# facebookresearch/fast3r

Hardware: AMD Instinct MI355X
Metric: views/sec (512^2, ViT-L) single forward pass at N=320 (higher is better)
Workload: dtype fp16

## Files before the change

### fast3r_amd/csrc/asm/attn_gen.py

```python
#!/usr/bin/env python3
import sys
import os

sys.path.insert(0, os.path.dirname(os.path.abspath(__file__)))
from isa import Program, Ins, Label, LabelRef, Lit, Neg, V, A, S, VCC, M0, EXEC, Reg

ARG_Q, ARG_O = 0, 8
ARG_LDQ = 16
ARG_NTILES = 32
ARG_QBS = 40
ARG_KVSHIFT = 56
ARG_STO = 64
ARG_KBS = 80
ARG_STLD = 96
ARG_TQ = 104
ARG_SEG = 112
SEG_BYTES = 24
ARG_DBG = ARG_SEG + 8 * SEG_BYTES
ARG_SCHED = ARG_DBG + 8
ARG_SIZE = ARG_SCHED + 32
FLAG_STATE_IN, FLAG_STATE_OUT = 1, 2

N_SLOTS = 4

s_q, s_k, s_vt, s_o = S(8, 2), S(10, 2), S(12, 2), S(14, 2)
s_ldq, s_ldk, s_ldvt, s_ldo = S(16), S(17), S(18), S(19)
s_nt, s_nseg = S(20), S(21)
s_wid, s_t, s_dma_u, s_seg_left = S(22), S(23), S(24), S(25)
s_kstep = S(26, 2)
s_m0base, s_seg, s_hopret, s_flags = S(28), S(29), S(30), S(31)
s_sto = S(32, 2)
s_lomask = S(34, 2)
s_ret, s_floor, s_ntm1 = S(36), S(37), S(38)
SEG0 = 52
s_stml = S(100, 2)


def seg_rec(i):
    return S(SEG0 + 6 * i, 2), S(SEG0 + 6 * i + 2, 2), S(SEG0 + 6 * i + 4)



s_delta = S(39)
s_shift = S(5)
s_tq = S(6)
s_rebase = S(7)
s_t0cyc, s_t0rt = S(SEG0 + 5), S(SEG0 + 11)

LANE = 0
s_mixrel = S(51)


class AttnGen:
    def __init__(self, dtype="f16", rowsum="pkadd", big_gap=None, k8_gap=2, name=None, ablate=(), cvt="rne", dma_aux="", dma_start=8, dma_step=None, pf=None, nslot=4,
                 fold="dot", head_dim=64, qk_planes=1, corr="f16", qk3_queues=True, k_hoist=True, qpw=None):
        assert dtype in ("f16", "bf16")
        assert head_dim in (64, 80, 128), "head widths with a generated kernel"
        assert qk_planes in (1, 2) and (qk_planes == 1 or (head_dim == 64 and dtype == "f16")) and corr in ("f16", "f8") and (corr == "f16" or qk_planes == 2)
        self.qk_planes, self.corr = qk_planes, corr
        self.qk3_queues = bool(qk3_queues)
        self.k_hoist = k_hoist
        self.dtype = dtype
        if rowsum == "pkadd" and dtype != "f16":
            rowsum = "add"
        self.rowsum = rowsum
        D = self.D = head_dim
        DK = self.DK = D * qk_planes
        assert qpw in (None, 2, 4) and (qpw is None or (head_dim == 64 and qk_planes == 1))
        self.QPW = QPW = qpw or (4 if (D == 64 and qk_planes == 1) else 2)
        self.WG_Q = 4 * QPW * 32
        self.NK = DK // 16
        self.QK_STEPS = ([(i, i) for i in range(self.NK)] if qk_planes == 1 else
                         [(i, i) for i in range(4)] + [(4 + i, i) for i in range(4)] + [(i, 4 + i) for i in range(4)])
        if corr == "f8":
            self.QK_STEPS = [(i, i) for i in range(4)] + [(6, 4, "f8", "unit", "lo"), (4, 6, "f8", "lo", "unit")]
        self.NQK = len(self.QK_STEPS)
        self.NDB = (D + 31) // 32
        self.DLAST = (D - 32 * (self.NDB - 1)) // 8
        self.KGROUPS = {64: [(0, 64)], 128: [(0, 64), (8192, 64)], 80: [(0, 64), (8192, 16)]}[DK]
        self.V_OFF = {64: 8192, 128: 16384, 80: 10240}[DK]
        self.SLOT = {64: 16384, 128: 32768, 80: 24576}[D] if qk_planes == 1 else 24576
        self.NP = 2 * (DK // 64) + (1 if D == 80 else 0) + 2 * (D // 64)
        if dma_step is None:
            dma_step = 6 if (D == 64 and qk_planes == 1 and self.QPW == 4) else 2
        self.dma_aux, self.dma_start, self.dma_step = dma_aux, dma_start, dma_step
        if pf is None:
            pf = 3 if corr == "f8" else 2
        assert nslot in (4, 8) and 2 <= pf <= nslot - 1
        assert D == 64 or nslot == 4
        self.pf, self.nslot = pf, nslot
        self.fold = fold
        self.LDS_X = nslot * self.SLOT
        self.lds_bytes = nslot * self.SLOT + 16
        v = 12
        self.S_BASE = v; v += 2 * QPW * 16
        self.P_BASE = v; v += QPW * 8
        self.NEGM = v; v += QPW * 16
        self.E_BASE = v; v += 4
        self.PSUM = v; v += QPW
        self.LRUN = v; v += QPW
        self.KCUR = v; v += 4
        self.VCUR = v; v += 4
        self.KREM = None
        if D == 80:
            self.KREM = v; v += 1
        self.SC_UNIT = self.SC_LO = None
        if corr == "f8":
            self.SC_UNIT = v; self.SC_LO = v + 1; v += 2
        a = 0
        self.O_BASE = a; a += QPW * self.NDB * 16
        self.Q_BASE = a; a += QPW * self.NK * 4
        self.KF_BASE = a; a += self.NK * 4
        self.VF_BASE = a; a += 2 * self.NDB * 4
        if a + self.NP <= 256:
            self.DOFF, self.doff_in_agpr = a, True
            a += self.NP
        else:
            self.DOFF, self.doff_in_agpr = v, False
            v += self.NP
        assert v <= 256 and a <= 256
        self.agpr_count = (a + 7) // 8 * 8
        pcs = []
        for goff, cols in self.KGROUPS:
            if cols == 64:
                pcs += [("A", "k", goff), ("A", "k", goff + 1024)]
        if D == 80:
            pcs.append(("A", "mix", None))
        for blk in range(D // 64):
            pcs += [("B", "vt", self.V_OFF + 8192 * blk), ("B", "vt", self.V_OFF + 8192 * blk + 1024)]
        assert len(pcs) == self.NP
        self.pieces = [(st, base, i, rel) for i, (st, base, rel) in enumerate(pcs)]
        if big_gap is None:
            big_gap = 4 if rowsum == "pkadd" else 5
        self.big_gap, self.k8_gap = (tuple(big_gap) if isinstance(big_gap, (tuple, list)) else (int(big_gap),)), k8_gap
        self.ablate = set(ablate)
        self.name = name or (f"f3r_attn_asm_q256_{dtype}" if (D == 64 and qk_planes == 1 and self.QPW == 2) else f"f3r_attn_asm_qk3f8_{dtype}" if corr == "f8" else f"f3r_attn_asm_qk3_{dtype}" if qk_planes == 2 else f"f3r_attn_asm_{dtype}" if D == 64 else f"f3r_attn_asm_d{D}_{dtype}")
        self.p = Program(self.name)
        if dtype == "f16":
            self.MFMA, self.MFMA8 = "v_mfma_f32_32x32x16_f16", "v_mfma_f32_32x32x8_f16"
            self.CVT, self.DOT, self.ONE2 = "v_cvt_pk_f16_f32", "v_dot2c_f32_f16", 0x3C003C00
            if cvt == "rtz":
                self.CVT = "v_cvt_pkrtz_f16_f32"
        else:
            self.MFMA, self.MFMA8 = "v_mfma_f32_32x32x16_bf16", "v_mfma_f32_32x32x8bf16_1k"
            self.CVT, self.DOT, self.ONE2 = "v_cvt_pk_bf16_f32", "v_dot2c_f32_bf16", 0x3F803F80

    def Sv(self, e, qb, r=None):
        base = self.S_BASE + e * self.QPW * 16 + qb * 16
        return V(base, 16) if r is None else V(base + r)

    def Pv(self, qb, ks, j=None):
        base = self.P_BASE + qb * 8 + ks * 4
        return V(base, 4) if j is None else V(base + j)

    def Nv(self, qb, r=None):
        base = self.NEGM + qb * 16
        return V(base, 16) if r is None else V(base + r)

    def Oa(self, qb, db, r=None):
        base = self.O_BASE + (qb * self.NDB + db) * 16
        return A(base, 16) if r is None else A(base + r)

    def Qa(self, qb, ds):
        return A(self.Q_BASE + (qb * self.NK + ds) * 4, 4)

    def KFa(self, ds):
        return A(self.KF_BASE + ds * 4, 4)

    def VFa(self, j):
# ... 244 lines not shown
            e("v_add_u32", V(6), S(40), V(6), comment="V^T row")
            e("v_lshrrev_b32", V(7), 1, V(6))
            e("v_and_b32", V(7), 7, V(7))
            e("v_xor_b32", V(7), V(7), V(10))
            e("v_lshlrev_b32", V(7), 4, V(7), comment="source chunk * 16")
            e("v_mul_lo_u32", V(6), V(6), s_ldvt)
            e("v_add_u32", V(6), V(6), V(7), comment="V^T rows 64..79: lane offset")
            e("s_cmp_lt_u32", s_wid, 2)
            e("s_cselect_b32", S(40), -1, 0)
            e("s_mov_b32", S(41), S(40))
            e("s_nop", 0)
            e("v_cndmask_b32", V(8), V(6), V(4), S(40, 2))
            park(mix, V(8))
            e("s_mov_b32", S(42), Lit(self.V_OFF + 8192 - 2048))
            e("s_cselect_b32", s_mixrel, Lit(self.KGROUPS[1][0]), S(42))
            e("s_lshl_b32", S(40), s_wid, 10)
            e("s_sub_u32", s_mixrel, s_mixrel, S(40), comment="destination of the mixed piece - s_m0base")
            for i in range(4):
                e("v_mov_b32", V(12 + i), 0)
            e("s_mul_i32", S(40), s_wid, Lit(self.SLOT))
            e("v_lshlrev_b32", V(8), 5, V(LANE))
            e("v_add_u32", V(8), S(40), V(8))
            e("ds_write_b128", V(8), V(12, 4), offset=self.V_OFF + 80 * 128)
            e("ds_write_b128", V(8), V(12, 4), offset=self.V_OFF + 80 * 128 + 16)
            e("s_waitcnt", "lgkmcnt(0)")
        e("s_lshl_b32", s_m0base, s_wid, 11, comment="slot 0 + wid * 2048")
        for i in range(self.pf):
            if i:
                e("s_add_u32", s_m0base, s_m0base, Lit(self.SLOT))
            self.emit_all(self.dma_pieces("A") + self.dma_pieces("B") + self.dma_advance())
            self.emit_all(self.seg_hop(i))
        e("s_add_u32", s_m0base, s_m0base, Lit(self.SLOT), comment="tile pf -> slot pf")
        self.emit_all(self.delta_for_tile())
        e("s_waitcnt", f"vmcnt({self.NP * (self.pf - 2)})", comment="tiles 0 and 1 have landed")
        e("s_barrier")
        for ds in range(NK):
            e_ = self.k_read(ds, 0)
            self.p.items.append(e_)
        e("s_waitcnt", "lgkmcnt(0)")
        self.emit_all(self.qk_mfmas(0))
        for ds in range(NK):
            self.p.items.append(self.k_read(ds, 1))

    def delta_for_tile(self):
        I = self.I
        msk = self.nslot - 1
        return [I("s_add_u32", S(40), s_t, 1), I("s_and_b32", S(40), S(40), msk), I("s_mov_b32", S(41), Lit((-msk * self.SLOT) & 0xFFFFFFFF)),
                I("s_cmp_eq_u32", S(40), 0), I("s_cselect_b32", s_delta, S(41), Lit(self.SLOT))]

    def own_rows_mask(self, qb):
        e = self.e
        e("s_sub_i32", S(46), s_shift, 32 * qb)
        e("v_cmp_le_i32", VCC, S(46), V(2))
        e("s_mov_b64", EXEC, VCC)

    def state_rows_offsets(self):
        e = self.e
        e("v_and_b32", V(2), 31, V(LANE), comment="lq")
        e("v_lshrrev_b32", V(3), 5, V(LANE), comment="g")
        e("s_load_dwordx2", S(44, 2), S(0, 2), Lit(ARG_STLD))
        e("s_waitcnt", "lgkmcnt(0)")
        e("v_mul_lo_u32", V(16), V(2), S(44))
        e("v_lshlrev_b32", V(1), 4, V(3))
        e("v_add_u32", V(16), V(16), V(1), comment="lq * st_o row stride + 16 g")
        e("v_mul_lo_u32", V(20), V(2), S(45))
        e("s_lshl_b32", S(46), S(44), 5)
        e("s_lshl_b32", S(47), S(45), 5)
# ... 34 lines not shown
            out += [I("s_nop", 0), I("global_load_lds_dwordx4", off, s_k if base == "k" else s_vt, **aux)]
        return out

    def dma_advance(self):
        I = self.I
        return [I("s_cmp_lt_u32", s_dma_u, s_ntm1),
                I("s_cselect_b32", S(40), s_kstep.sub(0), 0), I("s_cselect_b32", S(41), s_kstep.sub(1), 0),
                I("s_cselect_b32", S(42), 128, 0), I("s_cselect_b32", S(43), 1, 0),
                I("s_add_u32", s_k.sub(0), s_k.sub(0), S(40)), I("s_addc_u32", s_k.sub(1), s_k.sub(1), S(41)),
                I("s_add_u32", s_vt.sub(0), s_vt.sub(0), S(42)), I("s_addc_u32", s_vt.sub(1), s_vt.sub(1), 0),
                I("s_add_u32", s_dma_u, s_dma_u, S(43)),
                I("s_sub_u32", s_seg_left, s_seg_left, S(43))]

    def seg_hop(self, code):
        return [self.I("s_mov_b32", s_hopret, code), self.I("s_cmp_eq_u32", s_seg_left, 0), self.I("s_cbranch_scc1", self.L("NEXTSEG")),
                Label(f".L{self.name}_HOPRET_{code}")]

    def next_segment_block(self):
        e = self.e
        self.lab("NEXTSEG")
        e("s_add_u32", s_seg, s_seg, 1)
        for i in range(1, 8):
            e("s_cmp_eq_u32", s_seg, i)
            e("s_cbranch_scc1", self.L(f"SEG_{i}"))
        e("s_endpgm")
        for i in range(1, 8):
            k_i, vt_i, n_i = seg_rec(i)
            self.lab(f"SEG_{i}")
            e("s_mov_b64", s_k, k_i)
            e("s_mov_b64", s_vt, vt_i)
            e("s_mov_b32", s_seg_left, n_i)
            e("s_branch", self.L("SEG_DONE"))
        self.lab("SEG_DONE")
        for code in range(self.pf + 1):
            e("s_cmp_eq_u32", s_hopret, code)
            e("s_cbranch_scc1", self.L(f"HOPRET_{code}"))
        e("s_endpgm")

    def qk_mfmas(self, e_dst):
        out = []
        for step, st in enumerate(self.QK_STEPS):
            qf, kf = st[0], st[1]
            for qb in range(self.QPW):
                if len(st) == 2:
                    out.append(self.I(self.MFMA, self.Sv(e_dst, qb), self.KFa(kf), self.Qa(qb, qf), self.Nv(qb) if step == 0 else self.Sv(e_dst, qb)))
                else:
                    sc = {"unit": self.SC_UNIT, "lo": self.SC_LO}
                    out.append(self.I("v_mfma_scale_f32_32x32x64_f8f6f4", self.Sv(e_dst, qb), A(self.KF_BASE + kf * 4, 8), A(self.Q_BASE + (qb * self.NK + qf) * 4, 8),
                                      self.Sv(e_dst, qb), V(sc[st[3]]), V(sc[st[4]]), text="op_sel_hi:[0,0,0]"))
        return out

    def pv_mfmas(self, e_src=0):
        out = []
        for ks in range(2):
            for qb in range(self.QPW):
                for db in range(self.NDB):
                    out.append(self.I(self.MFMA, self.Oa(qb, db), self.VFa(ks * self.NDB + db), self.Pv(qb, ks), self.Oa(qb, db)))
        return out

    def softmax_flow(self, e):
        I = self.I
        QPW, NDB = self.QPW, self.NDB
        NPAIR = 8 * QPW
        flow = []
        first = 0 if QPW == 4 else 2
        E = lambda i, w: V(self.E_BASE + 2 * (i % 2) + w)

# ... 34 lines not shown
        if self.rowsum == "pkadd":
            red = ([I("v_pk_max_f16", V(1), V(PS), V(PS + 1)), I("v_pk_max_f16", V(2), V(PS + 2), V(PS + 3)), I("v_pk_max_f16", V(1), V(1), V(2))]
                   if self.QPW == 4 else [I("v_pk_max_f16", V(1), V(PS), V(PS + 1))])
            return [I("s_mov_b32", s_ret, ret_code)] + red + [
                    I("v_pk_max_f16", V(1), V(1), V(1), text="op_sel:[0,1] op_sel_hi:[1,0]"),
                    I("v_cmp_le_u32", VCC, Lit(0x50000000), V(1))] + ([] if "norare" in self.ablate else [
                    I("s_cbranch_vccnz", self.L(rare_label))])
        pad = [I("s_nop", 2)] if self.rowsum == "dot2c" else []
        red = ([I("v_max3_f32", V(1), V(PS), V(PS + 1), V(PS + 2)), I("v_max_f32", V(1), V(1), V(PS + 3))]
               if self.QPW == 4 else [I("v_max_f32", V(1), V(PS), V(PS + 1))])
        return [I("s_mov_b32", s_ret, ret_code)] + pad + red + [
                I("v_cmp_le_f32", VCC, 64.0, V(1))] + ([] if "norare" in self.ablate else [
                I("s_cbranch_vccnz", self.L(rare_label))])

    def l_adds(self):
        QPW, LRUN, PSUM = self.QPW, self.LRUN, self.PSUM
        if self.rowsum == "pkadd" and self.fold == "mix":
            out = []
            for half in (0, 1):
                for qb in range(QPW):
                    out.append(self.I("v_fma_mix_f32", V(LRUN + qb), V(PSUM + qb), 1.0, V(LRUN + qb),
                                      text=("op_sel:[1,0,0] " if half else "") + "op_sel_hi:[1,0,0]"))
            return out
        if self.rowsum == "pkadd":
            return [self.I(self.DOT, V(LRUN + qb), Lit(self.ONE2), V(PSUM + qb)) for qb in range(QPW)]
        return [self.I("v_add_f32", V(LRUN + qb), V(LRUN + qb), V(PSUM + qb)) for qb in range(QPW)]

    def addr_tail(self, is_a):
        I = self.I
        KCUR, VCUR = self.KCUR, self.VCUR
        regs = [KCUR + c for c in range(4)] + [VCUR, VCUR + 1] + ([self.KREM] if self.KREM is not None else []) if is_a else [VCUR + 2, VCUR + 3]
        return [I("v_add_u32", V(r), s_delta, V(r)) for r in regs]

    def stage(self, kind):
        I = self.I
        NK, NDB = self.NK, self.NDB
        is_a = kind.startswith("A")
        e_cur = 0 if is_a else 1
        e_nxt = 1 - e_cur
        has_qk = kind != "B_last"
        has_pv = kind != "A_first"
        do_sm = kind != "A_first"
        mf = (self.pv_mfmas() if has_pv else []) + (self.qk_mfmas(e_nxt) if has_qk else [])
        n_pv = 2 * self.QPW * NDB if has_pv else 0
        pinned = {i: [] for i in range(len(mf))}
        before = {i: [] for i in range(len(mf))}
        before[0].append(I("s_waitcnt", "lgkmcnt(0)"))
        hoist = self.corr == "f8" and self.qk3_queues and self.k_hoist
        if has_qk and has_pv:
            for ds in range(4 if hoist else 0, NK):
                pinned[ds - (4 if hoist else 0)].append(self.k_read(ds, 1 if is_a else 0))
            before[n_pv].append(I("s_waitcnt", "lgkmcnt(0)"))
        hoisted = [self.k_read(ds, 0 if is_a else 1) for ds in range(4)] if (hoist and has_qk) else []
        vbase = 0 if is_a else 2
        vreads = [I("ds_read_b128", self.VFa(ks * NDB + db), V(self.VCUR + vbase + ks), offset=db * 4096) for ks in range(2) for db in range(NDB)]
        tail = []
        if has_qk:
            for j, r in enumerate(vreads):
                pinned[n_pv + j].append(r)
        else:
            tail += vreads
        dma = (self.dma_pieces("A") if is_a else self.dma_pieces("B") + self.dma_advance()) if kind != "B_last" else []
        if "nodma" in self.ablate:
            dma = []
        tail += self.addr_tail(is_a)
        if kind == "B" and "nodma" not in self.ablate:
            tail += self.seg_hop(self.pf)
        flow = self.softmax_flow(e_cur) if do_sm else []
        if "nosoftmax" in self.ablate:
            flow = []
        two_queues = self.corr == "f8" and has_qk and has_pv and self.qk3_queues
        if not two_queues:
            flow = self.weave(flow, [(x, 0) for x in dma], start=self.dma_start, step=self.dma_step)
        if self.corr == "f8" and has_qk and has_pv and self.qk3_queues:
            n_last_read = n_pv + len(vreads)
            movable = [x for x in tail if getattr(x, "op", None) == "v_add_u32"]
            tail = [x for x in tail if getattr(x, "op", None) != "v_add_u32"]
            flow = flow + [(x, n_last_read) for x in movable]
            flow = flow + [(x, n_pv + 4 * self.QPW - 1) for x in hoisted]
            hoisted = []
        out = []
        fi = 0
        if two_queues:
            dq = list(dma)
            for i, m in enumerate(mf):
                out += before[i]
                out.append(m)
                took = len(pinned[i])
                out += pinned[i]
                cap = self.big_gap[i % len(self.big_gap)]
                if m.op.startswith("v_mfma_scale"):
                    cap = 2 * cap + 1
                gaps_left = len(mf) - i
                while took < cap:
                    flow_ok = fi < len(flow) and flow[fi][1] <= i
                    dma_due = dq and (not flow_ok or len(dq) > 3 * (gaps_left - 1))
                    if dma_due:
                        out.append(dq.pop(0))
                    elif flow_ok:
                        out.append(flow[fi][0])
# ... 225 lines not shown
        e("s_nop", 1)
        e("v_readfirstlane_b32", S(50), V(10))
        e("s_cmp_lt_u32", S(50), S(44))
        e("s_cbranch_scc0", self.L("F_EXIT"))
        e("s_mul_hi_u32", S(4), S(50), S(48))
        e("s_cmp_eq_u32", S(46), 1)
        e("s_cselect_b32", S(4), S(50), S(4), comment="z")
        e("s_mul_i32", S(51), S(4), S(46))
        e("s_sub_u32", S(51), S(50), S(51), comment="rem")
        e("s_mul_hi_u32", S(3), S(51), S(47))
        e("s_cmp_eq_u32", S(45), 1)
        e("s_cselect_b32", S(3), S(51), S(3), comment="y")
        e("s_mul_i32", S(2), S(3), S(45))
        e("s_sub_u32", S(2), S(51), S(2), comment="x")
        e("s_branch", self.L("WORK"))
        self.lab("F_EXIT")
        e("s_cmp_eq_u32", s_wid, 0)
        e("s_cbranch_scc0", self.L("F_END"))
        e("s_mov_b64", EXEC, 1)
        e("global_atomic_add", V(10), V(8), V(9), S(40, 2), offset=4, text="sc0")
        e("s_waitcnt", "vmcnt(0)")
        e("s_nop", 1)
        e("v_readfirstlane_b32", S(50), V(10))
        e("s_add_u32", S(50), S(50), 1)
        e("s_cmp_eq_u32", S(50), S(49))
        e("s_cbranch_scc0", self.L("F_END"))
        e("v_mov_b32", V(10), 0)
        e("v_mov_b32", V(11), 0)
        e("global_store_dwordx2", V(8), V(10, 2), S(40, 2), text="sc1")
        e("s_waitcnt", "vmcnt(0)")
        self.lab("F_END")
        e("s_endpgm")

    def build(self):
        p, e = self.p, self.e
        self.resume_labels = {0: [(0, "RESUME_A_FIRST"), (1, "RESUME_A")], 1: [(2, "RESUME_B"), (3, "RESUME_B_LAST")]}
        self.prologue()
        self.stage("A_first")
        e("s_mov_b32", s_ret, 0)
        e("s_branch", self.L("RARE_0"))
        self.lab("RESUME_A_FIRST")
        e("s_cmp_lt_u32", s_t, s_ntm1)
        e("s_cbranch_scc0", self.L("LAST_B"))
        p.items.append(Ins("s_nop", (0,), {}, "loop alignment"))
        self.lab("LOOP")
        self.stage("B")
        self.emit_all(self.check_block("RARE_1", 2))
        self.emit_all(self.l_adds())
        self.lab("RESUME_B")
        if "nobarrier" not in self.ablate:
            e("s_waitcnt", f"vmcnt({self.NP * (self.pf - 2)})")
            e("s_barrier")
        e("s_add_u32", s_t, s_t, 1)
        e("s_add_u32", S(40), s_t, self.pf)
        e("s_and_b32", S(40), S(40), self.nslot - 1)
        self.mul_const(S(40), S(40), self.SLOT)
        e("s_lshl_b32", S(41), s_wid, 11)
        e("s_add_u32", s_m0base, S(40), S(41), comment="LDS-DMA destination of tile t+pf")
        self.emit_all(self.delta_for_tile())
        self.stage("A")
        self.emit_all(self.check_block("RARE_0", 1))
        self.emit_all(self.l_adds())
        self.lab("RESUME_A")
        e("s_cmp_lt_u32", s_t, s_ntm1)
        e("s_cbranch_scc1", self.L("LOOP"))
        self.lab("LAST_B")
        self.stage("B_last")
        self.emit_all(self.check_block("RARE_1", 3))
        self.emit_all(self.l_adds())
        self.lab("RESUME_B_LAST")
        e("s_waitcnt", "lgkmcnt(0)")
        self.emit_all(self.pv_mfmas())
        self.epilogue()
        self.fetch_block()
        self.rare(0)
        self.rare(1)
        self.next_segment_block()
        return p

    def text(self):
        name = self.name
        body = self.p.body_text()
        return f"""
	.text
	.protected	{name}
	.globl	{name}
	.p2align	8
	.type	{name},@function
{name}:
{body}
.L{name}_end:
	.size	{name}, .L{name}_end-{name}
	.section	.rodata,"a",@progbits
	.p2align	6, 0x0
	.amdhsa_kernel {name}
		.amdhsa_group_segment_fixed_size {self.lds_bytes}
		.amdhsa_private_segment_fixed_size 0
		.amdhsa_kernarg_size {ARG_SIZE}
# ... 42 lines not shown
      - 2
      - 0
    .max_flat_workgroup_size: 256
    .name:           {self.name}
    .private_segment_fixed_size: 0
    .sgpr_count:     102
    .sgpr_spill_count: 0
    .symbol:         {self.name}.kd
    .uniform_work_group_size: 1
    .uses_dynamic_stack: false
    .vgpr_count:     {256 + self.agpr_count}
    .vgpr_spill_count: 0
    .wavefront_size: 64
"""


AttnGen2 = AttnGen


def module_text(gens):
    out = ['\t.amdgcn_target "amdgcn-amd-amdhsa--gfx950"\n\t.amdhsa_code_object_version 6\n']
    for g in gens:
        out.append(g.text())
    out.append("\t.amdgpu_metadata\n---\namdhsa.kernels:\n")
    for g in gens:
        out.append(g.metadata())
    out.append("amdhsa.target:   amdgcn-amd-amdhsa--gfx950\namdhsa.version:\n  - 1\n  - 2\n...\n\n\t.end_amdgpu_metadata\n")
    return "".join(out)


HEAD_DIMS = (64, 80, 128)


def product_generators(**kw):
    gens = []
    q3 = kw.pop("qk3_queues", True)
    kh = kw.pop("k_hoist", True)
    for hd in HEAD_DIMS:
        for dt in ("f16", "bf16"):
            g = AttnGen(dt, head_dim=hd, **kw)
            g.build()
            gens.append(g)
    kw3 = dict(kw)
    if kw3.get("dma_step") == 6:
        kw3["dma_step"] = None
    for dt in ("f16", "bf16"):
        g = AttnGen(dt, head_dim=64, qpw=2, **kw3)
        g.build()
        gens.append(g)
    for corr in ("f16", "f8"):
        g = AttnGen("f16", head_dim=64, qk_planes=2, corr=corr, qk3_queues=q3, k_hoist=kh, **kw3)
        g.build()
        gens.append(g)
    return gens


def main():
    import argparse
    ap = argparse.ArgumentParser()
    ap.add_argument("out")
    ap.add_argument("--rowsum", default="pkadd")
    ap.add_argument("--big-gap", default=None, help="fillers per MFMA gap: an int, or a comma list cycled over the gaps of a stage, e.g. 4,5")
    ap.add_argument("--k8-gap", type=int, default=2)
    ap.add_argument("--ablate", default="", help="comma list: nosoftmax,nodma,nobarrier,nolds,norare (timing only, wrong results)")
    ap.add_argument("--cvt", default="rne")
    ap.add_argument("--dma-aux", default="")
    ap.add_argument("--dma-start", type=int, default=8)
    ap.add_argument("--dma-step", type=int, default=6)
    ap.add_argument("--fold", default="dot")
    ap.add_argument("--layout", type=int, default=2, help="(accepted for old scripts; there is one layout)")
    ap.add_argument("--pf", type=int, default=None)
    ap.add_argument("--nslot", type=int, default=4)
    ap.add_argument("--qk3-queues", type=int, default=1, help="three-product kernels: 0 = in-order filler placement (measurement)")
    ap.add_argument("--k-hoist", type=int, default=1, help="fp8-correction kernel: 0 = K fragments requested in the stage that multiplies them (measurement)")
    a = ap.parse_args()
    bg = None if a.big_gap is None else (tuple(int(x) for x in a.big_gap.split(",")) if "," in a.big_gap else int(a.big_gap))
    gens = product_generators(rowsum=a.rowsum, big_gap=bg, k8_gap=a.k8_gap, ablate=[x for x in a.ablate.split(",") if x], cvt=a.cvt,
                              dma_aux=a.dma_aux, dma_start=a.dma_start, dma_step=a.dma_step, pf=a.pf, nslot=a.nslot, fold=a.fold, qk3_queues=bool(a.qk3_queues), k_hoist=bool(a.k_hoist))
    for g in gens:
        problems = g.p.check_hazards() if not a.ablate else []
        if problems:
            sys.stderr.write("\n".join(problems[:40]) + f"\n{len(problems)} hazard(s) in {g.name}\n")
            sys.exit(1)
    with open(a.out, "w") as f:
        f.write(module_text(gens))


if __name__ == "__main__":
    main()
```

### fast3r_amd/csrc/f3r_attn_asm.hip

```cpp
#include <cstddef>
#include <cstdlib>
#include <cstring>

#include "f3r_common.h"
#include "f3r_dispatch.h"

extern "C" const unsigned char f3r_attn_asm_hsaco[];
extern "C" const unsigned int f3r_attn_asm_hsaco_len;

namespace {

struct f3r_attn_asm_seg {
  const void* k;
  const void* vt;
  uint32_t tiles, pad;
};
struct f3r_attn_asm_args {
  const void* q;
  void* o;
  uint32_t ldq_b, ldk_b, ldvt_b, ldo_b;
  uint32_t n_tiles, n_seg;
  uint64_t q_bs, o_bs;
  uint32_t kv_shift, flags;
  float* st_o;
  float* st_ml;
  uint64_t k_bs, vt_bs;
  uint32_t st_o_ld_b, st_ml_ld_b;
  uint32_t tq, pad;
  f3r_attn_asm_seg seg[8];
  uint32_t* dbg;
  uint32_t* sched;
  uint32_t n_work, nx, nxy, nx_magic, nxy_magic, grid;
};
static_assert(sizeof(f3r_attn_asm_args) == 344 && offsetof(f3r_attn_asm_args, seg) == 112 && offsetof(f3r_attn_asm_args, dbg) == 304 &&
              offsetof(f3r_attn_asm_args, sched) == 312 && offsetof(f3r_attn_asm_args, n_work) == 320,
              "must match ARG_SIZE / ARG_SEG / ARG_DBG / ARG_SCHED of attn_gen.py");

constexpr int kNumHd = 3, kHd[kNumHd] = {64, 80, 128};
int hd_index(int hd) {
  for (int i = 0; i < kNumHd; ++i)
    if (kHd[i] == hd) return i;
  return -1;
}
AttnItem native_item(int hd, int planes) { return (hd == 64 && planes < 2) ? ATTN_ITEM_512 : ATTN_ITEM_256; }

F3rCodeObject<10> g_kernels = {f3r_attn_asm_hsaco,
                               {"f3r_attn_asm_f16", "f3r_attn_asm_bf16", "f3r_attn_asm_d80_f16", "f3r_attn_asm_d80_bf16", "f3r_attn_asm_d128_f16", "f3r_attn_asm_d128_bf16",
                                "f3r_attn_asm_qk3_f16", "f3r_attn_asm_qk3f8_f16", "f3r_attn_asm_q256_f16", "f3r_attn_asm_q256_bf16"}};

hipFunction_t get_fn(int dtype, int hi, int planes, AttnItem item) {
  if (dtype < 0 || dtype > 1 || hi < 0) return nullptr;
  const bool hd64 = kHd[hi] == 64;
  if (planes >= 2) return (hd64 && dtype == F3R_F16) ? g_kernels.get(4 + planes) : nullptr;
  if (item != native_item(kHd[hi], planes)) return hd64 ? g_kernels.get(8 + dtype) : nullptr;
  return g_kernels.get(2 * hi + dtype);
}

bool pow2(int x) { return x > 0 && (x & (x - 1)) == 0; }

bool q256_wins(int64_t tq, int64_t hb, int64_t cus) {
  const int64_t n512 = (tq + 511) / 512 * hb, n256 = (tq + 255) / 256 * hb;
  const double t512 = (double)((n512 + cus - 1) / cus), t256 = 0.64 * (double)((n256 + cus - 1) / cus);
  return t256 < 0.97 * t512;
}

int64_t tail_split_rows(int64_t tq, int64_t hb, int64_t cus) {
  const int64_t nqb = (tq + 511) / 512;
  if (nqb * hb <= cus) return 0;
  int64_t x = cus, y = hb;
  while (y) { const int64_t t = x % y; x = y; y = t; }
  const int64_t g = cus / x;
  const int64_t nqb_main = nqb / g * g;
  if (nqb_main == 0 || nqb_main == nqb) return 0;
  if (nqb_main * hb / cus > 8) return 0;
  const int64_t r = (nqb - nqb_main) * hb;
  if (2 * r > cus) return 0;
  return nqb_main * 512;
}

void plan_launches(const f3r_attn_args& a, AttnPlan& p) {
  const int hd = kHd[p.hd_index];
  p.main.rows = a.tq;
  p.main.item = native_item(hd, p.planes);
  if (p.main.item != ATTN_ITEM_512 || get_fn(a.dtype, p.hd_index, p.planes, ATTN_ITEM_256) == nullptr) return;
  static const char* force = getenv("F3R_ATTN_Q256");
  static const char* split = getenv("F3R_ATTN_TAIL_SPLIT");
  if (force && (force[0] == '0' || force[0] == '1')) {
    if (force[0] == '1') p.main.item = ATTN_ITEM_256;
    return;
  }
  const int64_t cus = f3r_device_cus(), hb = (int64_t)a.n_heads * a.batch;
  const bool may_split = !(split && split[0] == '0') && !a.state_in && !a.state_out && a.reserve_cus <= 0;
  const int64_t rows = may_split ? tail_split_rows(a.tq, hb, cus) : 0;
  if (rows > 0) {
    const AttnItem item = q256_wins(a.tq - rows, hb, cus) ? ATTN_ITEM_256 : ATTN_ITEM_512;
    if (a.tq - rows >= attn_item_wave_rows(item)) {
      p.main.rows = rows;
      p.tail.rows = a.tq - rows;
      p.tail.item = item;
      return;
    }
  }
  if (q256_wins(a.tq, hb, cus)) p.main.item = ATTN_ITEM_256;
}

}

bool f3r_attn_asm_plan(const f3r_attn_args& a, int64_t min_keys, AttnPlan* plan, const char** why) {
  *why = "";
  const int hd = a.head_dim == 0 ? 64 : a.head_dim;
  const int hi = hd_index(hd);
  if (hi < 0) { *why = "no generated kernel for this head_dim (64, 80, 128)"; return false; }
  const int qkp = a.qk_planes >= 2 ? a.qk_planes : 1;
  if (qkp >= 2 && (hd != 64 || a.dtype != F3R_F16)) { *why = "qk_planes 2 / 3 need head_dim 64 and fp16"; return false; }
  const int64_t wrows = attn_item_wave_rows(native_item(hd, qkp));
  if (a.causal) { *why = "causal mask"; return false; }
  if (!a.q_prescaled) { *why = "q not pre-scaled"; return false; }
  if (a.tq < wrows) { *why = "fewer query rows than one wave takes (128 at head_dim 64, 64 otherwise)"; return false; }
  if (a.kv_group > 1 && !pow2(a.kv_group)) { *why = "kv_group not a power of two"; return false; }
  if ((a.state_in || a.state_out) && a.batch != 1 && qkp < 2) { *why = "carried softmax state with batch > 1"; return false; }
  int first = -1;
  int64_t keys = 0;
  for (int s = 0; s < a.n_seg; ++s) {
    if (a.seg_len[s] == 0) continue;
    if (a.seg_len[s] % 64 != 0) { *why = "a K/V segment is not a multiple of 64 keys"; return false; }
    if (first < 0) first = s;
    if (a.ldvt[s] != a.ldvt[first] || a.k_batch_stride[s] != a.k_batch_stride[first] || a.vt_batch_stride[s] != a.vt_batch_stride[first]) {
      *why = "K/V segments with different ldvt / batch strides";
      return false;
    }
    keys += a.seg_len[s];
  }
  if (first < 0) { *why = "no keys"; return false; }
  if (keys < min_keys) { *why = "fewer keys than F3R_ATTN_ASM_MIN_KEYS"; return false; }
  if (keys / 64 >= (1ll << 31)) { *why = "too many keys"; return false; }
  if (wrows * a.ldq * 2 >= (1ll << 32) || wrows * a.ldo * 2 >= (1ll << 32) || 64 * a.ldk * 2 >= (1ll << 32) || (int64_t)hd * a.ldvt[first] * 2 >= (1ll << 32) ||
      wrows * a.n_heads * hd * 4 >= (1ll << 32)) {
    *why = "row strides too large for 32-bit lane offsets";
    return false;
  }
  if (a.tq >= (1ll << 31) || a.n_heads >= 65536 || a.batch >= 65536) { *why = "grid too large"; return false; }
  if (get_fn(a.dtype, hi, qkp, native_item(hd, qkp)) == nullptr) { *why = "the embedded code object could not be loaded on this device"; return false; }
  plan->family = ATTN_ASM;
  plan->hd_index = hi;
  plan->planes = qkp;
  plan_launches(a, *plan);
  return true;
}

const char* f3r_attn_asm_name(const f3r_attn_args& a, const AttnPlan& p) {
  const bool h = a.dtype == F3R_F16;
  if (p.planes == 2) return "f3r_attn_asm_qk3_f16 (hand-scheduled, three products per score block, csrc/asm/attn_gen.py)";
  if (p.planes == 3) return "f3r_attn_asm_qk3f8_f16 (hand-scheduled, three products per score block, the corrections on the fp8 MFMA, csrc/asm/attn_gen.py)";
  if (kHd[p.hd_index] == 80) return h ? "f3r_attn_asm_d80_f16 (hand-scheduled, csrc/asm/attn_gen.py)" : "f3r_attn_asm_d80_bf16 (hand-scheduled, csrc/asm/attn_gen.py)";
  if (kHd[p.hd_index] == 128) return h ? "f3r_attn_asm_d128_f16 (hand-scheduled, csrc/asm/attn_gen.py)" : "f3r_attn_asm_d128_bf16 (hand-scheduled, csrc/asm/attn_gen.py)";
  if (p.tail.rows > 0)
    return h ? "f3r_attn_asm_f16 + f3r_attn_asm_q256_f16 for the last round (hand-scheduled, csrc/asm/attn_gen.py)"
             : "f3r_attn_asm_bf16 + f3r_attn_asm_q256_bf16 for the last round (hand-scheduled, csrc/asm/attn_gen.py)";
  if (p.main.item == ATTN_ITEM_256)
    return h ? "f3r_attn_asm_q256_f16 (hand-scheduled, 256-query work items, csrc/asm/attn_gen.py)" : "f3r_attn_asm_q256_bf16 (hand-scheduled, 256-query work items, csrc/asm/attn_gen.py)";
  return h ? "f3r_attn_asm_f16 (hand-scheduled, csrc/asm/attn_gen.py)" : "f3r_attn_asm_bf16 (hand-scheduled, csrc/asm/attn_gen.py)";
}

static int launch_one(const f3r_attn_args& a, const AttnPlan& p, int64_t row0, const AttnAsmLaunch& l, hipStream_t stream) {
  const int hd = kHd[p.hd_index];
  const int wave_rows = attn_item_wave_rows(l.item);
  F3R_REQUIRE(l.rows >= wave_rows, "f3r_attn_fwd: a hand-scheduled launch of %lld query rows, fewer than the %d of one wave", (long long)l.rows, wave_rows);
  hipFunction_t fn = get_fn(a.dtype, p.hd_index, p.planes, l.item);
  if (!fn) {
    f3r_set_error("f3r_attn_fwd: the embedded hand-scheduled kernel could not be loaded on this device");
    return F3R_ERR_LAUNCH;
  }
  f3r_attn_asm_args k;
  memset(&k, 0, sizeof(k));
  k.q = (const char*)a.q + row0 * a.ldq * 2;
  k.o = (char*)a.o + row0 * a.ldo * 2;
  k.ldq_b = (uint32_t)(a.ldq * 2);
  k.ldk_b = (uint32_t)(a.ldk * 2);
  k.ldo_b = (uint32_t)(a.ldo * 2);
  k.q_bs = (uint64_t)a.q_batch_stride * 2;
  k.o_bs = (uint64_t)a.o_batch_stride * 2;
  int sh = 0;
  for (int gsz = a.kv_group > 1 ? a.kv_group : 1; gsz > 1; gsz >>= 1) ++sh;
  k.kv_shift = (uint32_t)sh;
  k.flags = (a.state_in ? 1u : 0u) | (a.state_out ? 2u : 0u);
  k.st_o = a.st_o;
  k.st_ml = a.st_ml;
  k.st_o_ld_b = (uint32_t)a.n_heads * (uint32_t)hd * 4u;
  k.st_ml_ld_b = (uint32_t)a.n_heads * 16u;
  k.tq = (uint32_t)l.rows;
  k.dbg = a.dbg_counters;
  for (int s = 0; s < a.n_seg; ++s) {
    if (a.seg_len[s] == 0) continue;
    f3r_attn_asm_seg& g = k.seg[k.n_seg++];
    g.k = a.k_seg[s];
    g.vt = a.vt_seg[s];
    g.tiles = (uint32_t)(a.seg_len[s] / 64);
    k.n_tiles += g.tiles;
    k.ldvt_b = (uint32_t)(a.ldvt[s] * 2);
    k.k_bs = (uint64_t)a.k_batch_stride[s] * 2;
    k.vt_bs = (uint64_t)a.vt_batch_stride[s] * 2;
// ... 40 lines not shown
```

### fast3r_amd/csrc/f3r_dispatch.h

```cpp
#pragma once
#include <atomic>
#include <map>
#include <mutex>

#include "f3r_common.h"

inline bool al16(const void* p) { return (((uintptr_t)p) & 15) == 0; }
inline bool al8(const void* p) { return (((uintptr_t)p) & 7) == 0; }

inline int f3r_device_cus() {
  static std::atomic<int> cache[64];
  int dev = 0, cu = 0;
  if (hipGetDevice(&dev) != hipSuccess) dev = 0;
  std::atomic<int>* slot = (dev >= 0 && dev < 64) ? &cache[dev] : nullptr;
  if (slot && (cu = slot->load(std::memory_order_relaxed)) != 0) return cu;
  if (hipDeviceGetAttribute(&cu, hipDeviceAttributeMultiprocessorCount, dev) != hipSuccess || cu < 8) cu = 256;
  if (slot) slot->store(cu, std::memory_order_relaxed);
  return cu;
}
inline int f3r_num_cus() { return f3r_device_cus() / 8 * 8; }

template <int N>
struct F3rCodeObject {
  const unsigned char* image;
// ... 64 lines not shown
  const int64_t rounds = (tiles + slots - 1) / slots;
  return eff * (float)tiles / (float)(rounds * slots);
}
inline float score_256(const f3r_gemm_args& a, int nh) {
  return tile_score(((a.M + 255) / 256) * ((a.N + 128 * nh - 1) / (128 * nh)), 256, nh == 2 ? 1.0f : 0.82f);
}
inline float score_128(const f3r_gemm_args& a) { return tile_score(((a.M + 127) / 128) * ((a.N + 127) / 128), 512, 0.72f); }

inline int f3r_gemm256_halves(const f3r_gemm_args& a, int forced) {
  if (a.epi == F3R_EPI_QKV) return 2;
  if (a.N % 256 != 0 || forced == 1) return 1;
  if (forced == 2) return 2;
  return score_256(a, 1) > score_256(a, 2) ? 1 : 2;
}
inline bool f3r_gemm256_preferred(const f3r_gemm_args& a) { return score_256(a, f3r_gemm256_halves(a, 0)) >= score_128(a); }

enum {
  ATTN_SEL_AUTO = 0,
  ATTN_SEL_HIP = 1,
  ATTN_SEL_ASM = 2,
};
enum AttnFamily {
  ATTN_HIP_CAUSAL,
  ATTN_HIP_BATCHED,
  ATTN_HIP,
  ATTN_GENERIC,
  ATTN_ASM,
};
enum AttnItem {
  ATTN_ITEM_512,
  ATTN_ITEM_256,
};
inline int attn_item_wave_rows(AttnItem item) { return item == ATTN_ITEM_512 ? 128 : 64; }
struct AttnAsmLaunch { int64_t rows = 0; AttnItem item = ATTN_ITEM_512; };
struct AttnPlan {
  AttnFamily family = ATTN_HIP;
  int hd_index = 0;
  int planes = 1;
  AttnAsmLaunch main, tail;
};
int f3r_attn_plan(const f3r_attn_args& a, AttnPlan* plan);
bool f3r_attn_asm_plan(const f3r_attn_args& a, int64_t min_keys, AttnPlan* plan, const char** why);
int f3r_attn_asm_launch(const f3r_attn_args& a, const AttnPlan& plan, hipStream_t stream);
const char* f3r_attn_asm_name(const f3r_attn_args& a, const AttnPlan& plan);
int f3r_attn_generic_launch(const f3r_attn_args& a, hipStream_t stream);
```

### include/f3r.h

```cpp
#ifndef F3R_H_
#define F3R_H_

#include <stddef.h>
#include <stdint.h>

#ifdef __cplusplus
extern "C" {
#endif

typedef void* f3r_stream_t;

typedef enum {
  F3R_OK = 0,
  F3R_ERR_ARG = -1,
  F3R_ERR_UNSUPPORTED = -2,
  F3R_ERR_LAUNCH = -3
} f3r_status;

typedef enum { F3R_F16 = 0, F3R_BF16 = 1 } f3r_dtype;
typedef enum { F3R_REAL_F32 = 0, F3R_REAL_F64 = 1 } f3r_real;
typedef enum { F3R_LOSS_DIS = 0, F3R_LOSS_LOG1P = 1 } f3r_loss_dis_mode;

#define F3R_MAX_SEG 8

// ... 86 lines not shown
  void* o;
  int64_t ldq, ldo;
  int64_t q_batch_stride, o_batch_stride;
  int64_t tq;
  int32_t batch;
  int32_t n_heads;
  int32_t n_seg;
  int32_t dtype;
  const void* k_seg[F3R_MAX_SEG];
  const void* vt_seg[F3R_MAX_SEG];
  int64_t seg_len[F3R_MAX_SEG];
  int64_t ldvt[F3R_MAX_SEG];
  int64_t ldk;
  int64_t k_batch_stride[F3R_MAX_SEG];
  int64_t vt_batch_stride[F3R_MAX_SEG];
  float scale;
  int32_t q_prescaled;
  float* st_o;
  float* st_ml;
  int32_t state_in;
  int32_t state_out;
  int32_t kv_group;
  int32_t causal;
  int64_t q_pos0;
  int64_t seg_pos0[F3R_MAX_SEG];
  int32_t kernel_sel;
  int32_t head_dim;
  uint32_t* dbg_counters;
  uint32_t* sched_counter;
  int32_t qk_planes;
  int32_t reserve_cus;
} f3r_attn_args;
#define F3R_ATTN_ASM_MIN_KEYS 2048

int f3r_attn_fwd(const f3r_attn_args* args, f3r_stream_t stream);
const char* f3r_attn_kernel_name(const f3r_attn_args* args);

int f3r_upsample2x(const void* in, const void* in_lo, void* out, void* out_lo, int batch, int h, int w, int C, int out_h, int out_w,
                   int dtype, f3r_stream_t stream);
int f3r_interp_bilinear(const void* in, const void* in_lo, void* out, void* out_lo, int batch, int h, int w, int C, int full_h, int full_w,
                        int out_h, int out_w, int dtype, f3r_stream_t stream);
int f3r_interp_bilinear_f8(const void* in, const void* in_lo, void* out, void* out_lo, void* out_f8, int batch, int h, int w, int C, int full_h,
                           int full_w, int out_h, int out_w, int dtype, f3r_stream_t stream);

typedef enum { F3R_DEPTH_EXP = 0, F3R_DEPTH_LINEAR = 1, F3R_DEPTH_SQUARE = 2 } f3r_depth_mode;
typedef enum { F3R_CONF_EXP = 0, F3R_CONF_SIGMOID = 1 } f3r_conf_mode;
int f3r_dpt_final(const void* x, const void* x_lo, const float* w, const float* b, int n_out, float* pts3d, float* conf, int64_t npix,
                  int Cin, int depth_mode, int conf_mode, float conf_vmin, float conf_vmax, int dtype, f3r_stream_t stream);

int f3r_cast_f32_to_lp(const float* in, void* out, void* out_lo, int64_t n, int dtype, f3r_stream_t stream);

size_t f3r_align_workspace_bytes(int n_prob);
int f3r_align_local_to_global(const float* conf, const float* pts_local, const float* pts_global, const uint8_t* valid_mask,
                              float* out, float* rts, float* thr_out, void* workspace, size_t ws_bytes, int n_prob,
                              int64_t npix, float quantile, f3r_stream_t stream);

size_t f3r_focal_workspace_bytes(int n_views, int H, int W);
int f3r_estimate_focal(const float* pts3d, const float* conf, float* focal, float* thr_out, void* workspace, size_t ws_bytes,
                       int n_views, int H, int W, float quantile, float ppx, float ppy, int n_iter, float min_focal, float max_focal,
                       f3r_stream_t stream);

size_t f3r_nn_index_bytes(int64_t m);
size_t f3r_nn_workspace_bytes(int64_t n);
int f3r_nn_build(const float* pts, int64_t m, void* index, size_t index_bytes, void* workspace, size_t ws_bytes, f3r_stream_t stream);
int f3r_nn_query(const void* index, const float* query, int64_t n, double* dist, int32_t* idx, void* workspace, size_t ws_bytes,
                 f3r_stream_t stream);
// ... 142 lines not shown
```

Before: 35.82.

## Add grouped attention kernel with one barrier per group of key tiles

```diff
diff --git a/fast3r_amd/csrc/asm/attn_gen.py b/fast3r_amd/csrc/asm/attn_gen.py
--- a/fast3r_amd/csrc/asm/attn_gen.py
+++ b/fast3r_amd/csrc/asm/attn_gen.py
@@ -53,7 +53,7 @@
 
 class AttnGen:
     def __init__(self, dtype="f16", rowsum="pkadd", big_gap=None, k8_gap=2, name=None, ablate=(), cvt="rne", dma_aux="", dma_start=8, dma_step=None, pf=None, nslot=4,
-                 fold="dot", head_dim=64, qk_planes=1, corr="f16", qk3_queues=True, k_hoist=True, qpw=None):
+                 fold="dot", head_dim=64, qk_planes=1, corr="f16", qk3_queues=True, k_hoist=True, qpw=None, tiles_per_barrier=1):
         assert dtype in ("f16", "bf16")
         assert head_dim in (64, 80, 128), "head widths with a generated kernel"
         assert qk_planes in (1, 2) and (qk_planes == 1 or (head_dim == 64 and dtype == "f16")) and corr in ("f16", "f8") and (corr == "f16" or qk_planes == 2)
@@ -86,8 +86,12 @@
         self.dma_aux, self.dma_start, self.dma_step = dma_aux, dma_start, dma_step
         if pf is None:
             pf = 3 if corr == "f8" else 2
-        assert nslot in (4, 8) and 2 <= pf <= nslot - 1
+            if tiles_per_barrier > 1:
+                pf = tiles_per_barrier + 1
+        G = self.G = int(tiles_per_barrier)
+        assert nslot in (4, 8) and G >= 1 and G + 1 <= pf and pf + G <= nslot, "LDS ring: G + 1 <= pf (read after write) and pf + G <= nslot (write after read)"
         assert D == 64 or nslot == 4
+        assert G == 1 or (D == 64 and qk_planes == 1 and self.QPW == 4)
         self.pf, self.nslot = pf, nslot
         self.fold = fold
         self.LDS_X = nslot * self.SLOT
@@ -135,6 +139,8 @@
         self.big_gap, self.k8_gap = (tuple(big_gap) if isinstance(big_gap, (tuple, list)) else (int(big_gap),)), k8_gap
         self.ablate = set(ablate)
         self.name = name or (f"f3r_attn_asm_q256_{dtype}" if (D == 64 and qk_planes == 1 and self.QPW == 2) else f"f3r_attn_asm_qk3f8_{dtype}" if corr == "f8" else f"f3r_attn_asm_qk3_{dtype}" if qk_planes == 2 else f"f3r_attn_asm_{dtype}" if D == 64 else f"f3r_attn_asm_d{D}_{dtype}")
+        if name is None and G > 1:
+            self.name += "_grp"
         self.p = Program(self.name)
         if dtype == "f16":
             self.MFMA, self.MFMA8 = "v_mfma_f32_32x32x16_f16", "v_mfma_f32_32x32x8_f16"
@@ -445,7 +451,10 @@
             self.emit_all(self.seg_hop(i))
         e("s_add_u32", s_m0base, s_m0base, Lit(self.SLOT), comment="tile pf -> slot pf")
         self.emit_all(self.delta_for_tile())
-        e("s_waitcnt", f"vmcnt({self.NP * (self.pf - 2)})", comment="tiles 0 and 1 have landed")
+        if self.G == 1:
+            e("s_waitcnt", f"vmcnt({self.NP * (self.pf - 2)})", comment="tiles 0 and 1 have landed")
+        else:
+            e("s_waitcnt", f"vmcnt({self.NP * (self.pf - 1 - self.G)})", comment=f"tiles 0 .. {self.G} have landed")
         e("s_barrier")
         for ds in range(NK):
             e_ = self.k_read(ds, 0)
@@ -546,7 +555,7 @@
             e("s_mov_b32", s_seg_left, n_i)
             e("s_branch", self.L("SEG_DONE"))
         self.lab("SEG_DONE")
-        for code in range(self.pf + 1):
+        for code in range(self.pf + self.G):
             e("s_cmp_eq_u32", s_hopret, code)
             e("s_cbranch_scc1", self.L(f"HOPRET_{code}"))
         e("s_endpgm")
@@ -647,7 +656,7 @@
         regs = [KCUR + c for c in range(4)] + [VCUR, VCUR + 1] + ([self.KREM] if self.KREM is not None else []) if is_a else [VCUR + 2, VCUR + 3]
         return [I("v_add_u32", V(r), s_delta, V(r)) for r in regs]
 
-    def stage(self, kind):
+    def stage(self, kind, hop_code=None):
         I = self.I
         NK, NDB = self.NK, self.NDB
         is_a = kind.startswith("A")
@@ -680,7 +689,7 @@
             dma = []
         tail += self.addr_tail(is_a)
         if kind == "B" and "nodma" not in self.ablate:
-            tail += self.seg_hop(self.pf)
+            tail += self.seg_hop(self.pf if hop_code is None else hop_code)
         flow = self.softmax_flow(e_cur) if do_sm else []
         if "nosoftmax" in self.ablate:
             flow = []
@@ -972,17 +981,8 @@
         self.lab("F_END")
         e("s_endpgm")
 
-    def build(self):
-        p, e = self.p, self.e
-        self.resume_labels = {0: [(0, "RESUME_A_FIRST"), (1, "RESUME_A")], 1: [(2, "RESUME_B"), (3, "RESUME_B_LAST")]}
-        self.prologue()
-        self.stage("A_first")
-        e("s_mov_b32", s_ret, 0)
-        e("s_branch", self.L("RARE_0"))
-        self.lab("RESUME_A_FIRST")
-        e("s_cmp_lt_u32", s_t, s_ntm1)
-        e("s_cbranch_scc0", self.L("LAST_B"))
-        p.items.append(Ins("s_nop", (0,), {}, "loop alignment"))
+    def plain_loop(self):
+        e = self.e
         self.lab("LOOP")
         self.stage("B")
         self.emit_all(self.check_block("RARE_1", 2))
@@ -1004,6 +1004,55 @@
         self.lab("RESUME_A")
         e("s_cmp_lt_u32", s_t, s_ntm1)
         e("s_cbranch_scc1", self.L("LOOP"))
+
+    def grouped_loop(self):
+        e = self.e
+        G = self.G
+        self.lab("LOOP")
+        for k in range(G):
+            code_a, code_b = (1, 2) if k == 0 else (2 + 2 * k, 3 + 2 * k)
+            self.stage("B", hop_code=self.pf + k)
+            self.emit_all(self.check_block("RARE_1", code_b))
+            self.emit_all(self.l_adds())
+            self.lab("RESUME_B" if k == 0 else f"RESUME_B_{k}")
+            if k == G - 1 and "nobarrier" not in self.ablate:
+                e("s_waitcnt", f"vmcnt({self.NP * (self.pf - 1 - G)})", comment=f"this wave's pieces of tiles .. t+1+{G} have landed")
+                e("s_barrier")
+            e("s_add_u32", s_t, s_t, 1)
+            e("s_add_u32", S(40), s_t, self.pf)
+            e("s_and_b32", S(40), S(40), self.nslot - 1)
+            self.mul_const(S(40), S(40), self.SLOT)
+            e("s_lshl_b32", S(41), s_wid, 11)
+            e("s_add_u32", s_m0base, S(40), S(41), comment="LDS-DMA destination of tile t+pf")
+            self.emit_all(self.delta_for_tile())
+            self.stage("A")
+            self.emit_all(self.check_block("RARE_0", code_a))
+            self.emit_all(self.l_adds())
+            self.lab("RESUME_A" if k == 0 else f"RESUME_A_{k}")
+            e("s_cmp_lt_u32", s_t, s_ntm1)
+            if k < G - 1:
+                e("s_cbranch_scc0", self.L("LAST_B"))
+            else:
+                e("s_cbranch_scc1", self.L("LOOP"))
+
+    def build(self):
+        p, e = self.p, self.e
+        self.resume_labels = {0: [(0, "RESUME_A_FIRST"), (1, "RESUME_A")], 1: [(2, "RESUME_B"), (3, "RESUME_B_LAST")]}
+        for k in range(1, self.G):
+            self.resume_labels[0].append((2 + 2 * k, f"RESUME_A_{k}"))
+            self.resume_labels[1].append((3 + 2 * k, f"RESUME_B_{k}"))
+        self.prologue()
+        self.stage("A_first")
+        e("s_mov_b32", s_ret, 0)
+        e("s_branch", self.L("RARE_0"))
+        self.lab("RESUME_A_FIRST")
+        e("s_cmp_lt_u32", s_t, s_ntm1)
+        e("s_cbranch_scc0", self.L("LAST_B"))
+        p.items.append(Ins("s_nop", (0,), {}, "loop alignment"))
+        if self.G > 1:
+            self.grouped_loop()
+        else:
+            self.plain_loop()
         self.lab("LAST_B")
         self.stage("B_last")
         self.emit_all(self.check_block("RARE_1", 3))
@@ -1112,13 +1161,16 @@
 HEAD_DIMS = (64, 80, 128)
 
 
-def product_generators(**kw):
+GROUPED_RING = dict(tiles_per_barrier=2, pf=4, nslot=8)
+
+
+def product_generators(ring=None, **kw):
     gens = []
     q3 = kw.pop("qk3_queues", True)
     kh = kw.pop("k_hoist", True)
     for hd in HEAD_DIMS:
         for dt in ("f16", "bf16"):
-            g = AttnGen(dt, head_dim=hd, **kw)
+            g = AttnGen(dt, head_dim=hd, **(dict(kw, name=f"f3r_attn_asm_{dt}", **ring) if (ring and hd == 64) else kw))
             g.build()
             gens.append(g)
     kw3 = dict(kw)
@@ -1130,6 +1182,10 @@
         gens.append(g)
     for corr in ("f16", "f8"):
         g = AttnGen("f16", head_dim=64, qk_planes=2, corr=corr, qk3_queues=q3, k_hoist=kh, **kw3)
+        g.build()
+        gens.append(g)
+    for dt in ("f16", "bf16"):
+        g = AttnGen(dt, head_dim=64, **dict(kw, name=f"f3r_attn_asm_{dt}_grp", **(ring or GROUPED_RING)))
         g.build()
         gens.append(g)
     return gens
@@ -1149,13 +1205,19 @@
     ap.add_argument("--dma-step", type=int, default=6)
     ap.add_argument("--fold", default="dot")
     ap.add_argument("--layout", type=int, default=2, help="(accepted for old scripts; there is one layout)")
-    ap.add_argument("--pf", type=int, default=None)
-    ap.add_argument("--nslot", type=int, default=4)
+    ap.add_argument("--pf", type=int, default=None, help="tiles the LDS-DMA runs ahead (with --tiles-per-barrier / --nslot 8: of the 512-query head_dim-64 kernels only)")
+    ap.add_argument("--nslot", type=int, default=4, help="LDS ring slots; 8: the 512-query head_dim-64 kernels only (the other slots do not fit eight times)")
+    ap.add_argument("--tiles-per-barrier", type=int, default=None,
+                    help="G: one s_barrier per G key tiles in every 512-query head_dim-64 kernel of the module, the _grp symbols included (1 with --nslot 4: all of them the plain form)")
     ap.add_argument("--qk3-queues", type=int, default=1, help="three-product kernels: 0 = in-order filler placement (measurement)")
     ap.add_argument("--k-hoist", type=int, default=1, help="fp8-correction kernel: 0 = K fragments requested in the stage that multiplies them (measurement)")
     a = ap.parse_args()
     bg = None if a.big_gap is None else (tuple(int(x) for x in a.big_gap.split(",")) if "," in a.big_gap else int(a.big_gap))
-    gens = product_generators(rowsum=a.rowsum, big_gap=bg, k8_gap=a.k8_gap, ablate=[x for x in a.ablate.split(",") if x], cvt=a.cvt,
+    ring = None
+    if a.tiles_per_barrier is not None or a.nslot == 8:
+        ring = dict(tiles_per_barrier=a.tiles_per_barrier or 1, pf=a.pf, nslot=a.nslot)
+        a.pf, a.nslot = None, 4
+    gens = product_generators(ring=ring, rowsum=a.rowsum, big_gap=bg, k8_gap=a.k8_gap, ablate=[x for x in a.ablate.split(",") if x], cvt=a.cvt,
                               dma_aux=a.dma_aux, dma_start=a.dma_start, dma_step=a.dma_step, pf=a.pf, nslot=a.nslot, fold=a.fold, qk3_queues=bool(a.qk3_queues), k_hoist=bool(a.k_hoist))
     for g in gens:
         problems = g.p.check_hazards() if not a.ablate else []
diff --git a/fast3r_amd/csrc/f3r_attn_asm.hip b/fast3r_amd/csrc/f3r_attn_asm.hip
--- a/fast3r_amd/csrc/f3r_attn_asm.hip
+++ b/fast3r_amd/csrc/f3r_attn_asm.hip
@@ -44,15 +44,17 @@
 }
 AttnItem native_item(int hd, int planes) { return (hd == 64 && planes < 2) ? ATTN_ITEM_512 : ATTN_ITEM_256; }
 
-F3rCodeObject<10> g_kernels = {f3r_attn_asm_hsaco,
+F3rCodeObject<12> g_kernels = {f3r_attn_asm_hsaco,
                                {"f3r_attn_asm_f16", "f3r_attn_asm_bf16", "f3r_attn_asm_d80_f16", "f3r_attn_asm_d80_bf16", "f3r_attn_asm_d128_f16", "f3r_attn_asm_d128_bf16",
-                                "f3r_attn_asm_qk3_f16", "f3r_attn_asm_qk3f8_f16", "f3r_attn_asm_q256_f16", "f3r_attn_asm_q256_bf16"}};
-
-hipFunction_t get_fn(int dtype, int hi, int planes, AttnItem item) {
+                                "f3r_attn_asm_qk3_f16", "f3r_attn_asm_qk3f8_f16", "f3r_attn_asm_q256_f16", "f3r_attn_asm_q256_bf16", "f3r_attn_asm_f16_grp",
+                                "f3r_attn_asm_bf16_grp"}};
+
+hipFunction_t get_fn(int dtype, int hi, int planes, AttnItem item, bool grouped = false) {
   if (dtype < 0 || dtype > 1 || hi < 0) return nullptr;
   const bool hd64 = kHd[hi] == 64;
   if (planes >= 2) return (hd64 && dtype == F3R_F16) ? g_kernels.get(4 + planes) : nullptr;
   if (item != native_item(kHd[hi], planes)) return hd64 ? g_kernels.get(8 + dtype) : nullptr;
+  if (grouped) return hd64 ? g_kernels.get(10 + dtype) : nullptr;
   return g_kernels.get(2 * hi + dtype);
 }
 
@@ -78,7 +80,7 @@
   return nqb_main * 512;
 }
 
-void plan_launches(const f3r_attn_args& a, AttnPlan& p) {
+void plan_items(const f3r_attn_args& a, AttnPlan& p) {
   const int hd = kHd[p.hd_index];
   p.main.rows = a.tq;
   p.main.item = native_item(hd, p.planes);
@@ -102,6 +104,12 @@
     }
   }
   if (q256_wins(a.tq, hb, cus)) p.main.item = ATTN_ITEM_256;
+}
+
+void plan_launches(const f3r_attn_args& a, int64_t keys, AttnPlan& p) {
+  plan_items(a, p);
+  if (kHd[p.hd_index] != 64 || p.planes != 1 || keys < F3R_ATTN_GROUPED_MIN_KEYS) return;
+  p.main.grouped = p.main.item == ATTN_ITEM_512;
 }
 
 }
@@ -144,7 +152,7 @@
   plan->family = ATTN_ASM;
   plan->hd_index = hi;
   plan->planes = qkp;
-  plan_launches(a, *plan);
+  plan_launches(a, keys, *plan);
   return true;
 }
 
@@ -154,11 +162,17 @@
   if (p.planes == 3) return "f3r_attn_asm_qk3f8_f16 (hand-scheduled, three products per score block, the corrections on the fp8 MFMA, csrc/asm/attn_gen.py)";
   if (kHd[p.hd_index] == 80) return h ? "f3r_attn_asm_d80_f16 (hand-scheduled, csrc/asm/attn_gen.py)" : "f3r_attn_asm_d80_bf16 (hand-scheduled, csrc/asm/attn_gen.py)";
   if (kHd[p.hd_index] == 128) return h ? "f3r_attn_asm_d128_f16 (hand-scheduled, csrc/asm/attn_gen.py)" : "f3r_attn_asm_d128_bf16 (hand-scheduled, csrc/asm/attn_gen.py)";
+  if (p.tail.rows > 0 && p.main.grouped)
+    return h ? "f3r_attn_asm_f16_grp + f3r_attn_asm_q256_f16 for the last round (hand-scheduled, one barrier per group of key tiles, csrc/asm/attn_gen.py)"
+             : "f3r_attn_asm_bf16_grp + f3r_attn_asm_q256_bf16 for the last round (hand-scheduled, one barrier per group of key tiles, csrc/asm/attn_gen.py)";
   if (p.tail.rows > 0)
     return h ? "f3r_attn_asm_f16 + f3r_attn_asm_q256_f16 for the last round (hand-scheduled, csrc/asm/attn_gen.py)"
              : "f3r_attn_asm_bf16 + f3r_attn_asm_q256_bf16 for the last round (hand-scheduled, csrc/asm/attn_gen.py)";
   if (p.main.item == ATTN_ITEM_256)
     return h ? "f3r_attn_asm_q256_f16 (hand-scheduled, 256-query work items, csrc/asm/attn_gen.py)" : "f3r_attn_asm_q256_bf16 (hand-scheduled, 256-query work items, csrc/asm/attn_gen.py)";
+  if (p.main.grouped)
+    return h ? "f3r_attn_asm_f16_grp (hand-scheduled, one barrier per group of key tiles, csrc/asm/attn_gen.py)"
+             : "f3r_attn_asm_bf16_grp (hand-scheduled, one barrier per group of key tiles, csrc/asm/attn_gen.py)";
   return h ? "f3r_attn_asm_f16 (hand-scheduled, csrc/asm/attn_gen.py)" : "f3r_attn_asm_bf16 (hand-scheduled, csrc/asm/attn_gen.py)";
 }
 
@@ -166,7 +180,7 @@
   const int hd = kHd[p.hd_index];
   const int wave_rows = attn_item_wave_rows(l.item);
   F3R_REQUIRE(l.rows >= wave_rows, "f3r_attn_fwd: a hand-scheduled launch of %lld query rows, fewer than the %d of one wave", (long long)l.rows, wave_rows);
-  hipFunction_t fn = get_fn(a.dtype, p.hd_index, p.planes, l.item);
+  hipFunction_t fn = get_fn(a.dtype, p.hd_index, p.planes, l.item, l.grouped);
   if (!fn) {
     f3r_set_error("f3r_attn_fwd: the embedded hand-scheduled kernel could not be loaded on this device");
     return F3R_ERR_LAUNCH;
diff --git a/fast3r_amd/csrc/f3r_dispatch.h b/fast3r_amd/csrc/f3r_dispatch.h
--- a/fast3r_amd/csrc/f3r_dispatch.h
+++ b/fast3r_amd/csrc/f3r_dispatch.h
@@ -120,7 +120,11 @@
   ATTN_ITEM_256,
 };
 inline int attn_item_wave_rows(AttnItem item) { return item == ATTN_ITEM_512 ? 128 : 64; }
-struct AttnAsmLaunch { int64_t rows = 0; AttnItem item = ATTN_ITEM_512; };
+struct AttnAsmLaunch {
+  int64_t rows = 0;
+  AttnItem item = ATTN_ITEM_512;
+  bool grouped = false;
+};
 struct AttnPlan {
   AttnFamily family = ATTN_HIP;
   int hd_index = 0;
diff --git a/include/f3r.h b/include/f3r.h
--- a/include/f3r.h
+++ b/include/f3r.h
@@ -142,6 +142,7 @@
   int32_t reserve_cus;
 } f3r_attn_args;
 #define F3R_ATTN_ASM_MIN_KEYS 2048
+#define F3R_ATTN_GROUPED_MIN_KEYS 8192
 
 int f3r_attn_fwd(const f3r_attn_args* args, f3r_stream_t stream);
 const char* f3r_attn_kernel_name(const f3r_attn_args* args);
```

Result: faster. 36.25 (median of 6 runs) (+1.2%).
